# NikNazarov/TorchPIV

Hardware: AMD Instinct MI355X
Metric: image-pairs/sec at 4 MP, wind=64 ov=32 2-pass CWS; % HBM roofline (higher is better)
Workload: dtype u32 exact sums + f64 / f32

## Files before the change

torchpiv_amd/csrc/xcorr_tile.hpp:

```cpp
#pragma once
#include <hip/hip_runtime.h>
#include <stdint.h>

#include "fft_inreg.hpp"
#include "piv_kernels.h"

namespace tpiv {

template <int WS, bool PLANAR_ = false>
struct TileGeo {
    static constexpr int WPW = 64 / WS;
    static constexpr int TS = WS > 32 ? 32 : WS;
    static constexpr int PITCH = TS + 1;
    static constexpr int NT = 64 / TS;
    static constexpr int TILE = TS * PITCH;
    static constexpr bool PLANAR = PLANAR_;
    static constexpr int HROWS = WS / 2 + 1;
    static constexpr int HTILE = HROWS * PITCH;
    static constexpr int LDS_FLOATS = NT * TILE * (PLANAR ? 1 : 2);
    static constexpr int MAP_PITCH = WS + 1;
    static constexpr int NDW = WS / 4;
};

template <int CTRL>
// ... 709 lines not shown
                if (ci < CG::T) {
                    pa[j * CG::PITCH4 + part] = make_uint4(raw.ca[k][0], raw.ca[k][1], raw.ca[k][2], raw.ca[k][3]);
                    pb[j * CG::PITCH4 + part] = make_uint4(raw.cb[k][0], raw.cb[k][1], raw.cb[k][2], raw.cb[k][3]);
                }
            }
            wave_sync();
            const int rlo = -8, rhi = p.H + 7;
            const float gy0f = (float)g.y0;
            const int base_a = clamp_i(f2i_sat_t(floorf(gy0f - vy)), rlo, rhi);
            const int base_b = clamp_i(f2i_sat_t(floorf(gy0f + vy)), rlo, rhi);
            const uint4* s0 = pa + (clamp_i(c.dya, rlo, rhi) - base_a) * CG::PITCH4;
            const uint4* s1 = pa + (clamp_i(c.uya, rlo, rhi) - base_a) * CG::PITCH4;
            const uint4* s2 = pb + (clamp_i(c.dyb, rlo, rhi) - base_b) * CG::PITCH4;
            const uint4* s3 = pb + (clamp_i(c.uyb, rlo, rhi) - base_b) * CG::PITCH4;
            auto fetch = [&](const uint4* src, uint32_t (&d)[NB]) TPIV_LAMBDA_INLINE {
#pragma unroll
                for (int q = 0; q < NB / 4; ++q) {
                    const uint4 t = src[q];
                    d[4 * q] = t.x, d[4 * q + 1] = t.y, d[4 * q + 2] = t.z, d[4 * q + 3] = t.w;
                }
                static_assert(CG::RPG * 4 >= NB, "patch rows hold the whole 16-byte unit of the last dword");
                d[NB - 1] = read_unit_x(src + NB / 4);
            };
            if (raw.fix) {
                constexpr int LAST = CG::LOADED / 4 - 1;
                auto fix_lds = [&](const uint4* src, int cls) TPIV_LAMBDA_INLINE {
                    if (cls != 0) {
                        const uint32_t* sw = reinterpret_cast<const uint32_t*>(src);
                        const uint32_t px = (cls == 1 ? (sw[0] & 0xffu) : (sw[LAST] >> 24)) * 0x01010101u;
                        uint4* dst = const_cast<uint4*>(src);
#pragma unroll
                        for (int q = 0; q < CG::RPG; ++q) dst[q] = make_uint4(px, px, px, px);
                    }
                };
                fix_lds(s0, raw.cls & 3);
                fix_lds(s1, (raw.cls >> 2) & 3);
                fix_lds(s2, (raw.cls >> 4) & 3);
                fix_lds(s3, (raw.cls >> 6) & 3);
                wave_sync();
            }
            constexpr bool LAZY = FAST && WS == 64;
            if constexpr (LAZY) {
                lz0 = s0, lz1 = s1, lz2 = s2, lz3 = s3;
            } else {
                fetch(s0, ra0);
                fetch(s1, ra1);
                fetch(s2, rb0);
                fetch(s3, rb1);
            }
            float4* wbuf = reinterpret_cast<float4*>(lds + CG::FLOATS) + (lane / WS) * (WS + 1);
            {
                const float gxf = gx0f + (float)r;
                const float nxa = gxf - vx, nxb = gxf + vx;
                const float uxa_f = ceilf(nxa), dxa_f = floorf(nxa);
                const float uxb_f = ceilf(nxb), dxb_f = floorf(nxb);
                wave_sync();
                wbuf[r] = make_float4(uxa_f - nxa, nxa - dxa_f, uxb_f - nxb, nxb - dxb_f);
                wave_sync();
            }
            if constexpr (FAST) {
                constexpr bool LAZY = WS == 64;
                auto pull = [&](auto qc) TPIV_LAMBDA_INLINE {
                    constexpr int q = decltype(qc)::value;
                    auto one = [&](const uint4* src, uint32_t (&d)[NB]) TPIV_LAMBDA_INLINE {
                        if constexpr (4 * q + 3 < NB) {
                            const uint4 t = src[q];
                            d[4 * q] = t.x, d[4 * q + 1] = t.y, d[4 * q + 2] = t.z, d[4 * q + 3] = t.w;
                        } else {
                            d[NB - 1] = read_unit_x(src + NB / 4);
                        }
                    };
                    one(lz0, ra0), one(lz1, ra1), one(lz2, rb0), one(lz3, rb1);
                };
                if constexpr (LAZY) {
                    pull(std::integral_constant<int, 0>{});
                    pull(std::integral_constant<int, 1>{});
                }
                auto row_lerp = [&](auto kc, const uint32_t (&r0_)[NB], const uint32_t (&r1_)[NB], float wu_, float wd_) TPIV_LAMBDA_INLINE {
                    constexpr int k = decltype(kc)::value;
                    return fmaf(byte_f<k, NB>(r1_), wd_, byte_f<k, NB>(r0_) * wu_);
                };
                float va = row_lerp(std::integral_constant<int, 0>{}, ra0, ra1, c.wya_up, c.wya_dn);
                float vb = row_lerp(std::integral_constant<int, 0>{}, rb0, rb1, c.wyb_up, c.wyb_dn);
                static_for<0, WS>([&](auto kc) TPIV_LAMBDA_INLINE {
                    constexpr int k = decltype(kc)::value;
                    if constexpr (k % 8 == 0 && k > 0) __builtin_amdgcn_sched_barrier(0);
                    if constexpr (LAZY && k % 16 == 0 && k > 0) pull(std::integral_constant<int, k / 16 + 1>{});
                    const float4 wx = wbuf[k];
                    const float na = row_lerp(std::integral_constant<int, k + 1>{}, ra0, ra1, c.wya_up, c.wya_dn);
                    const float nb = row_lerp(std::integral_constant<int, k + 1>{}, rb0, rb1, c.wyb_up, c.wyb_dn);
#ifdef TPIV_MUTANT_LERP
                    x[k].x = fmaf(na, wx.y * 1.001f, va * wx.x);
#else
                    x[k].x = fmaf(na, wx.y, va * wx.x);
#endif
                    x[k].y = fmaf(nb, wx.w, vb * wx.z);
                    va = na;
                    vb = nb;
                });
            } else {
            unsigned dmask_a = c.ydeg_a ? ~0u : 0u, dmask_b = c.ydeg_b ? ~0u : 0u;
            asm volatile("" : "+v"(dmask_a), "+v"(dmask_b));
            static_for<0, WS>([&](auto kc) TPIV_LAMBDA_INLINE {
                constexpr int k = decltype(kc)::value;
                if constexpr (k % 8 == 0 && k > 0) __builtin_amdgcn_sched_barrier(0);
                const float4 wx = wbuf[k];
                x[k].x = bilerp_ref_m(byte_f<k, NB>(ra0), byte_f<k + 1, NB>(ra0), byte_f<k, NB>(ra1),
                                      byte_f<k + 1, NB>(ra1), wx.x, wx.y, c.wya_up, c.wya_dn, dmask_a);
                x[k].y = bilerp_ref_m(byte_f<k, NB>(rb0), byte_f<k + 1, NB>(rb0), byte_f<k, NB>(rb1),
                                      byte_f<k + 1, NB>(rb1), wx.z, wx.w, c.wyb_up, c.wyb_dn, dmask_b);
            });
            }
            wave_sync();
        } else {
            wave_sync();
            static_for<0, RBH>([&](auto hc) TPIV_LAMBDA_INLINE {
            constexpr int k0 = decltype(hc)::value * RBL;
#pragma unroll UNR_CWS
            for (int k = 0; k < RBL; ++k) {
                const float nxa = (gx0f + (float)(k0 + k)) - vx;
                const float uxa_f = ceilf(nxa), dxa_f = floorf(nxa);
                const int uxa = f2i_sat_t(uxa_f), dxa = f2i_sat_t(dxa_f);
                rowbuf[k] = bilerp_ref(fetch_clamped_t(fa, (long long)c.dya * p.W + dxa, HW),
                                       fetch_clamped_t(fa, (long long)c.dya * p.W + uxa, HW),
                                       fetch_clamped_t(fa, (long long)c.uya * p.W + dxa, HW),
                                       fetch_clamped_t(fa, (long long)c.uya * p.W + uxa, HW), uxa_f - nxa,
                                       nxa - dxa_f, c.wya_up, c.wya_dn, c.ydeg_a || (uxa == dxa));
            }
#pragma unroll
            for (int k = 0; k < RBL; ++k) x[k0 + k].x = rowbuf[k];
#pragma unroll UNR_CWS
            for (int k = 0; k < RBL; ++k) {
                const float nxb = (gx0f + (float)(k0 + k)) + vx;
                const float uxb_f = ceilf(nxb), dxb_f = floorf(nxb);
                const int uxb = f2i_sat_t(uxb_f), dxb = f2i_sat_t(dxb_f);
                rowbuf[k] = bilerp_ref(fetch_clamped_t(fb, (long long)c.dyb * p.W + dxb, HW),
                                       fetch_clamped_t(fb, (long long)c.dyb * p.W + uxb, HW),
                                       fetch_clamped_t(fb, (long long)c.uyb * p.W + dxb, HW),
                                       fetch_clamped_t(fb, (long long)c.uyb * p.W + uxb, HW), uxb_f - nxb,
                                       nxb - dxb_f, c.wyb_up, c.wyb_dn, c.ydeg_b || (uxb == dxb));
            }
#pragma unroll
            for (int k = 0; k < RBL; ++k) x[k0 + k].y = rowbuf[k];
            });
            wave_sync();
        }
        sa = 0.f;
        sb = 0.f;
        if constexpr (!FAST) {
#pragma unroll
            for (int k = 0; k < WS; ++k) {
                sa += x[k].x;
                sb += x[k].y;
            }
        }
    }
}

template <int WS>
__device__ __forceinline__ unsigned long long exclusion_row_mask(int m, int ys, int wv) {
    static_assert(WS <= 64, "one 64-bit mask per row");
    const int my_ = m / WS, mx_ = m % WS, KD = WS * WS;
    const int dj = ys - my_;
    unsigned long long ex = 0ull;
    auto span = [&](int lo_, int hi_) TPIV_LAMBDA_INLINE {
        lo_ = lo_ < 0 ? 0 : lo_;
        hi_ = hi_ > WS - 1 ? WS - 1 : hi_;
        if (lo_ > hi_) return 0ull;
        const unsigned long long ones = (hi_ - lo_ + 1) >= 64 ? ~0ull : ((1ull << (hi_ - lo_ + 1)) - 1ull);
        return ones << lo_;
    };
    if (dj >= -wv && dj <= wv) ex |= span(mx_ - wv, mx_ + wv);
    if (dj + 1 >= -wv && dj + 1 <= wv) ex |= span(mx_ - wv + WS, mx_ + wv + WS);
    if (dj - 1 >= -wv && dj - 1 <= wv) ex |= span(mx_ - wv - WS, mx_ + wv - WS);
    if (ys == 0 && (m - wv - wv * WS) <= 0) ex |= 1ull;
    if (ys == WS - 1 && (m + wv + wv * WS) >= KD - 1) ex |= 1ull << (WS - 1);
    return ex;
}

__device__ __forceinline__ float max3_skip_nan(float a, float b, float c) {
    float o;
    asm("v_max3_f32 %0, %1, %2, %3" : "=v"(o) : "v"(a), "v"(b), "v"(c));
    return o;
}
__device__ __forceinline__ float max_skip_nan(float a, float b) {
    float o;
    asm("v_max_f32 %0, %1, %2" : "=v"(o) : "v"(a), "v"(b));
    return o;
}

template <int WS, bool PLANAR, bool SCALED = false>
__device__ __forceinline__ void peak_analysis(const PassParams& p, const float (&row)[WS], float* tile, int w, int r,
                                              bool active, bool dead, size_t fidx, float scale = 1.0f) {
    using G = TileGeo<WS, PLANAR>;
    constexpr bool SMALLMAP = G::WPW * WS * G::MAP_PITCH > G::LDS_FLOATS;
    static_assert(G::WPW * 3 * G::MAP_PITCH <= G::LDS_FLOATS, "map rows must fit the tile LDS");
    float* my_map = tile + w * ((SMALLMAP ? 3 : WS) * G::MAP_PITCH);
    const int ys = (r + WS / 2) % WS;
    float cmin = 3.4e38f, rraw = -3.4e38f;
#pragma unroll
    for (int k = 0; k < WS; ++k) {
        cmin = fminf(cmin, row[k]);
        rraw = fmaxf(rraw, row[k]);
    }
    cmin = grp_min<WS>(cmin);
    const float ncs = -(cmin * scale);
    auto shifted = [&](float c_) TPIV_LAMBDA_INLINE {
        if constexpr (SCALED) return __fadd_rn(fmaf(c_, scale, ncs), 1e-7f);
        else return __fadd_rn(__fsub_rn(c_, cmin), 1e-7f);
    };
    if constexpr (!SMALLMAP) {
        static_for<0, WS>([&](auto kc) TPIV_LAMBDA_INLINE {
            constexpr int xsft = decltype(kc)::value;
            my_map[ys * G::MAP_PITCH + xsft] = row[(xsft + WS / 2) % WS];
        });
    }
    const float rmax = shifted(rraw);
    const float gmax = grp_reduce<WS>(rmax, [](float a, float b) TPIV_LAMBDA_INLINE { return fmaxf(a, b); });
    auto imin = [](int a, int b) TPIV_LAMBDA_INLINE { return a < b ? a : b; };
    const int ywin = grp_reduce<WS>(rmax == gmax ? ys : WS - 1, imin);
    const int row0 = SMALLMAP ? ywin - 1 : 0;
    if constexpr (SMALLMAP) {
        wave_sync();
        const int slot = ys - row0;
        if (slot >= 0 && slot <= 2) {
            static_for<0, WS>([&](auto kc) TPIV_LAMBDA_INLINE {
                constexpr int xsft = decltype(kc)::value;
                my_map[slot * G::MAP_PITCH + xsft] = row[(xsft + WS / 2) % WS];
            });
        }
    }
    wave_sync();

    if (p.dbg_corr != nullptr && active) {
        int yy = ys;
        asm volatile("" : "+v"(yy));
        float* d = p.dbg_corr + fidx * WS * WS + yy * WS;
        static_for<0, WS>([&](auto kc) TPIV_LAMBDA_INLINE {
            constexpr int xsft = decltype(kc)::value;
            d[xsft] = shifted(row[(xsft + WS / 2) % WS]);
        });
    }
    const int xwin = grp_reduce<WS>(shifted(my_map[(ywin - row0) * G::MAP_PITCH + r]) == gmax ? r : WS - 1, imin);

    const int m = ywin * WS + xwin;
    const int KD = WS * WS;
    const int wv = p.val_win;
    float sraw;
    {
        const unsigned long long ex = exclusion_row_mask<WS>(m, ys, wv);
        const int exl = (int)(unsigned)ex, exh = (int)(unsigned)(ex >> 32);
        float acc = __int_as_float(-1);
        static_for<0, WS / 2>([&](auto kc) TPIV_LAMBDA_INLINE {
            constexpr int x0 = 2 * decltype(kc)::value, x1 = x0 + 1;
            const int k0 = __builtin_amdgcn_sbfe(x0 < 32 ? exl : exh, x0 & 31, 1);
            const int k1 = __builtin_amdgcn_sbfe(x1 < 32 ? exl : exh, x1 & 31, 1);
            const float v0 = __int_as_float(__float_as_int(row[(x0 + WS / 2) % WS]) | k0);
            const float v1 = __int_as_float(__float_as_int(row[(x1 + WS / 2) % WS]) | k1);
            acc = max3_skip_nan(acc, v0, v1);
        });
        sraw = acc;
    }
    sraw = grp_reduce<WS>(sraw, [](float a, float b) TPIV_LAMBDA_INLINE { return max_skip_nan(a, b); });
    const float second_v = sraw != sraw ? gmax : shifted(sraw);

    {
        int left = m + 1, right = m - 1, top = m + WS, bot = m - WS;
        if (left >= KD - 1) left = m;
        if (right <= 0) right = m;
        if (top >= KD - 1) top = m;
        if (bot <= 0) bot = m;
        int q = m;
        q = (r == 1) ? left : q;
        q = (r == 2) ? right : q;
        q = (r == 3) ? top : q;
        q = (r == 4) ? bot : q;
        float outv = shifted(my_map[(q / WS - row0) * G::MAP_PITCH + (q % WS)]);
        outv = (r == 5) ? second_v : outv;
        outv = (r == 6) ? __int_as_float(m) : outv;
        outv = (r == 7) ? __int_as_float(dead ? 1 : 0) : outv;
        if (r < 8 && active) p.peak_raw[fidx * 8 + r] = outv;
    }
}



template <int WS>
__device__ __forceinline__ void peak_candidates(const PassParams& p, const float (&row)[WS], float* tile, int w, int r,
                                                bool active, bool dead, size_t fidx, float band_abs) {
    static_assert(WS == 8 || WS == 16 || WS == 32 || WS == 64, "64 / WS windows per wavefront");
    auto wballot = [&](bool pred) TPIV_LAMBDA_INLINE {
        const unsigned long long b_ = __ballot(pred);
        if constexpr (WS == 64) return b_;
        else return (b_ >> (w * WS)) & ((1ull << WS) - 1ull);
    };
    auto any_left = [](unsigned long long mk) TPIV_LAMBDA_INLINE {
        if constexpr (WS == 64) return mk != 0ull;
        else return __ballot(mk != 0ull) != 0ull;
    };
    auto mine_left = [](unsigned long long mk) TPIV_LAMBDA_INLINE {
        if constexpr (WS == 64) return true;
        else return mk != 0ull;
    };
    float* const my_row = tile + w * WS;
    const int ys = (r + WS / 2) % WS;
    if (p.dbg_corr != nullptr && active) {
        int yy = ys;
        asm volatile("" : "+v"(yy));
        float* d = p.dbg_corr + fidx * WS * WS + yy * WS;
        static_for<0, WS>([&](auto kc) TPIV_LAMBDA_INLINE {
            constexpr int xsft = decltype(kc)::value;
            d[xsft] = row[(xsft + WS / 2) % WS];
        });
    }
    float rmin = 3.4e38f, rmax = -3.4e38f;
#pragma unroll
    for (int k = 0; k < WS; ++k) {
        rmin = fminf(rmin, row[k]);
        rmax = fmaxf(rmax, row[k]);
    }
    const float cmin = grp_min<WS>(rmin);
    const float gmax = grp_reduce<WS>(rmax, [](float a, float b) TPIV_LAMBDA_INLINE { return fmaxf(a, b); });
    const float band = fmaxf(p.exact_band_range * (gmax - cmin), band_abs);
    bool open = !(band > 0.0f) || !(gmax > cmin);
    auto park = [&](int rl) TPIV_LAMBDA_INLINE {
        wave_sync();
        if (r == rl) {
#pragma unroll
            for (int k = 0; k < WS; ++k) my_row[(k + WS / 2) % WS] = row[k];
        }
        wave_sync();
        return my_row[r];
    };
    auto row_of_lane = [](int rl) TPIV_LAMBDA_INLINE { return (rl + WS / 2) % WS; };
    int m = 0;
    {
        const unsigned long long rows = wballot(rmax >= gmax - band);
        open = open || __popcll(rows) != 1;
        const int rl = rows ? (int)__builtin_ctzll(rows) : 0;
        const unsigned long long cols = wballot(park(rl) >= gmax - band);
        open = open || __popcll(cols) != 1;
        m = row_of_lane(rl) * WS + (cols ? (int)__builtin_ctzll(cols) : 0);
    }
    const int wv = p.val_win;
    int s[EXACT_MAX_SECOND] = {-1, -1, -1};
    {
        const unsigned long long ex = exclusion_row_mask<WS>(m, ys, wv);
        const int exl = (int)(unsigned)ex, exh = (int)(unsigned)(ex >> 32);
        int smax = -1;
        static_for<0, WS>([&](auto kc) TPIV_LAMBDA_INLINE {
            constexpr int xsft = decltype(kc)::value;
            constexpr int xo = (xsft + WS / 2) % WS;
            const int kill = __builtin_amdgcn_sbfe(xsft < 32 ? exl : exh, xsft & 31, 1);
            const int cnd = __float_as_int(__fsub_rn(row[xo], cmin)) | kill;
            smax = cnd > smax ? cnd : smax;
        });
        const int sall = grp_reduce<WS>(smax, [](int a, int b) TPIV_LAMBDA_INLINE { return a > b ? a : b; });
        const float thr = __int_as_float(sall) - band;
        unsigned long long rows = sall >= 0 ? wballot(smax >= 0 && __int_as_float(smax) >= thr) : 0ull;
        open = open || __popcll(rows) > EXACT_MAX_SECOND;
        int ns = 0;
        for (int it = 0; it < EXACT_MAX_SECOND; ++it) {
            if (!any_left(rows)) break;
            const bool on = mine_left(rows);
            const int rl = on ? (int)__builtin_ctzll(rows) : 0;
            rows &= rows - 1;
            const int yr = row_of_lane(rl);
            const unsigned long long exr = exclusion_row_mask<WS>(m, yr, wv);
            unsigned long long cols = wballot(__fsub_rn(park(rl), cmin) >= thr) & ~exr;
            cols = on ? cols : 0ull;
            for (int k = 0; k < WS; ++k) {
                if (!any_left(cols)) break;
                const bool has = mine_left(cols);
                const int q = yr * WS + (has ? (int)__builtin_ctzll(cols) : 0);
                cols &= cols - 1;
                s[0] = (has && ns == 0) ? q : s[0];
                s[1] = (has && ns == 1) ? q : s[1];
                s[2] = (has && ns == 2) ? q : s[2];
                ns += has ? 1 : 0;
            }
        }
        open = open || ns > EXACT_MAX_SECOND;
    }
    int n[EXACT_MAX_MIN] = {-1, -1, -1, -1};
    {
        const float thr = cmin + band;
        unsigned long long rows = wballot(rmin <= thr);
        bool over = __popcll(rows) > EXACT_MAX_MIN;
        int nn = 0;
        for (int it = 0; it < EXACT_MAX_MIN; ++it) {
            if (!any_left(rows)) break;
            const bool on = mine_left(rows);
            const int rl = on ? (int)__builtin_ctzll(rows) : 0;
            rows &= rows - 1;
            const int yr = row_of_lane(rl);
            unsigned long long cols = wballot(park(rl) <= thr);
            cols = on ? cols : 0ull;
            over = over || nn + __popcll(cols) > EXACT_MAX_MIN;
            for (int k = 0; k < EXACT_MAX_MIN; ++k) {
                if (!any_left(cols)) break;
                const bool has = mine_left(cols) && cols != 0ull && nn < EXACT_MAX_MIN;
                const int q = yr * WS + (cols ? (int)__builtin_ctzll(cols) : 0);
                cols &= cols - 1;
                n[0] = (has && nn == 0) ? q : n[0];
                n[1] = (has && nn == 1) ? q : n[1];
                n[2] = (has && nn == 2) ? q : n[2];
                n[3] = (has && nn == 3) ? q : n[3];
                nn += has ? 1 : 0;
            }
        }
        n[3] = over ? -2 : n[3];
    }
    if (r == 0 && active) {
        const int m_out = dead ? -2 : (open ? -1 : m);
        auto pack = [](int lo_, int hi_) TPIV_LAMBDA_INLINE { return ((unsigned)lo_ & 0xffffu) | ((unsigned)hi_ << 16); };
        uint4 rec;
        rec.x = pack(m_out, s[0]);
        rec.y = pack(s[1], s[2]);
        rec.z = pack(n[0], n[1]);
        rec.w = pack(n[2], n[3]);
        p.cand[fidx] = rec;
    }
}

template <int WS, int MODE, int OCC, bool FAST, bool CAND, int ROLE = 0>
__device__ __forceinline__ void xcorr_tile_body(const PassParams& p) {
    constexpr bool PLANAR = OCC > 2;
    using G = TileGeo<WS, PLANAR>;
    static_assert(WS == 8 || WS == 16 || WS == 32 || WS == 64, "tile sizes of this kernel");
    constexpr int RBH = 64 * (WS + 1) <= G::LDS_FLOATS ? 1 : 2;
    static_assert(MODE == MODE_PASS1 || 64 * (WS / RBH + 1) <= G::LDS_FLOATS,
                  "slow-path row buffer (shifted passes) must fit the tile LDS");
    constexpr int LDSF = (MODE == MODE_CWS && CoopGeo<WS>::LDS_FLOATS > G::LDS_FLOATS)
                             ? CoopGeo<WS>::LDS_FLOATS : G::LDS_FLOATS;
    __shared__ __attribute__((aligned(16))) float tile[LDSF];

    using TW = std::conditional_t<WS == 16, TwRegs<WS>, TwLiteral>;
    TW tw;
    if constexpr (!std::is_same<TW, TwLiteral>::value) tw.init();

    const int N = p.n_rows * p.n_cols;
    const int groups = (N + G::WPW - 1) / G::WPW;
    const bool listed = ROLE == 0 && MODE != MODE_PASS1 && p.list_mode != 0;
    const int items = listed ? __builtin_amdgcn_readfirstlane((int)*p.slow_count) : p.batch * groups;
    const int st = p.ws - p.ov;
    auto real_item = [&](int pos) TPIV_LAMBDA_INLINE { return listed ? __builtin_amdgcn_readfirstlane(p.slow_list[pos]) : pos; };

    constexpr int QCH = WS <= 16 ? 4 : 1;
    const int xcd = blockIdx.x & 7;
    const int chunk = (int)(((long long)items + 7) / 8);
    const int lo = __builtin_amdgcn_readfirstlane(xcd * chunk < items ? xcd * chunk : items);
    const int hi = __builtin_amdgcn_readfirstlane(items - lo > chunk ? lo + chunk : items);
    unsigned* const ctr = p.work_ctr + xcd * 16;
    int q_base = 0;
    int q_left = 0;
    auto q_issue = [&]() TPIV_LAMBDA_INLINE -> unsigned {
        unsigned v = 0;
        if (QCH == 1 || q_left == 0) {
            if (fresh_lane() == 0) v = atomicAdd(ctr, (unsigned)QCH);
        }
        return v;
    };
    auto q_take = [&](unsigned q_raw) TPIV_LAMBDA_INLINE -> int {
        if (QCH == 1 || q_left == 0) {
            const unsigned v = (unsigned)__builtin_amdgcn_readfirstlane((int)q_raw);
            q_base = v < (unsigned)(hi - lo) ? lo + (int)v : hi;
            q_left = QCH;
        }
        const int it = q_base + (QCH - q_left);
        --q_left;
        return it;
    };

    auto geom_of = [&](int pos, int w) TPIV_LAMBDA_INLINE {
        ItemGeom g;
        const int item = real_item(pos);
        g.pair = fast_div(item, p.groups_magic, p.groups_shift);
        const int gi = item - g.pair * groups;
        const int win_raw = gi * G::WPW + w;
        g.active = win_raw < N ? 1 : 0;
        g.win = g.active ? win_raw : N - 1;
        const int wrow = fast_div(g.win, p.ncols_magic, p.ncols_shift);
        g.y0 = wrow * st;
        g.x0 = (g.win - wrow * p.n_cols) * st;
        g.fidx = (size_t)g.pair * N + g.win;
        return g;
    };
    auto shift_of = [&](const ItemGeom& g, float& vx, float& vy) TPIV_LAMBDA_INLINE {
        if constexpr (MODE == MODE_PASS1) {
            vx = 0.f;
            vy = 0.f;
        } else {
            if constexpr (MODE == MODE_CWS) {
                pred_half_shift_cws_f32(p, g.fidx, vx, vy);
            } else {
                double sx, sy;
                pred_half_shift<MODE>(p, g.fidx, sx, sy);
                vx = (float)sx;
                vy = (float)sy;
            }
        }
    };

    int item = q_take(q_issue());
    if (item >= hi) return;
    int nitem = q_take(q_issue());
    constexpr bool RECOMPUTE = WS >= 32;
    float vx, vy;
    RawRows<WS, MODE> raw;
    ItemGeom gcur;
    CoopOff<WS> coff;
    if constexpr (MODE == MODE_CWS) coff.init(fresh_lane() % WS, p.W);
    {
        const int l0 = fresh_lane();
        gcur = geom_of(item, l0 / WS);
        shift_of(gcur, vx, vy);
        issue_rows<WS, MODE, FAST>(p, gcur, l0 % WS, vx, vy, raw, coff);
    }

    TPIV_STAMP_DECL
    TPIV_STAMP_START;
    for (int nnitem; item < hi; item = nitem, nitem = nnitem) {
        const unsigned q_raw = q_issue();
#ifdef TPIV_STAMPS
        ++st_iter;
#endif
        const int lane = fresh_lane();
        const int w = lane / WS;
        const int r = lane % WS;
        const ItemGeom g = RECOMPUTE ? geom_of(item, w) : gcur;
        const bool active = g.active != 0;
        const size_t fidx = g.fidx;
        const int nit = nitem < hi ? nitem : item;
        const ItemGeom gnext = geom_of(nit, w);
        float nvx, nvy;
        shift_of(gnext, nvx, nvy);

        if constexpr (ROLE == 1) {
            if (!raw.reg) {
                if (lane == 0) p.slow_list[atomicAdd(p.slow_count, 1u)] = item;
                nnitem = q_take(q_raw);
                issue_rows<WS, MODE, FAST>(p, gnext, r, nvx, nvy, raw, coff);
                vx = nvx;
                vy = nvy;
                if constexpr (!RECOMPUTE) gcur = gnext;
                continue;
            }
        }
        cf x[WS];
        float sa, sb;
        constexpr int NBS = WS >= 32 ? G::WPW : 1;
        int band_s[NBS];
        TPIV_STAMP(0);
        RowSquares sq;
        convert_rows<WS, MODE, RBH, FAST, CAND, ROLE == 1 ? 1 : 0>(p, g, r, lane, vx, vy, raw, x, sa, sb, tile, &sq);
        TPIV_STAMP(1);
        if constexpr (WS >= 64) nnitem = q_take(q_raw);
        if constexpr (WS <= 32) issue_rows<WS, MODE, FAST>(p, gnext, r, nvx, nvy, raw, coff);

        if (p.dbg_win != nullptr && active) {
            int rr = r;
            asm volatile("" : "+v"(rr));
            float* d = p.dbg_win + fidx * 2 * WS * WS + rr * WS;
#pragma unroll
            for (int k = 0; k < WS; ++k) {
                d[k] = x[k].x;
                d[WS * WS + k] = x[k].y;
            }
        }

        bool dead = false;
        float end_scale = 1.0f;
        constexpr bool FASTN = FAST && MODE != MODE_PASS1;
        constexpr bool NOSWAP = WS == 64 && !(MODE == MODE_DWS && FAST);
        auto up_sign = []() TPIV_LAMBDA_INLINE { return fresh_lane() >= 32 ? 0x80000000u : 0u; };
        auto sflip = [](float v, unsigned sg) TPIV_LAMBDA_INLINE { return __uint_as_float(__float_as_uint(v) ^ sg); };
        if constexpr (!FASTN) {
            sa = grp_sum<WS>(sa);
            sb = grp_sum<WS>(sb);
            const float ma = sa * (1.0f / (WS * WS)), mb = sb * (1.0f / (WS * WS));
            float ka = 1.f, kb = 1.f;
            if constexpr (MODE == MODE_PASS1) {
                dead = (sa == 0.f) || (sb == 0.f);
                ka = dead ? 0.f : 1.0f / ma;
                kb = dead ? 0.f : 1.0f / mb;
            }
            if constexpr (CAND) {
                auto uadd = [](unsigned a_, unsigned b_) TPIV_LAMBDA_INLINE { return a_ + b_; };
                const unsigned saa = grp_reduce<WS>(sq.aa, uadd), sbb = grp_reduce<WS>(sq.bb, uadd);
                constexpr double NN = (double)(WS * WS);
                const double da = (double)sa, db = (double)sb;
                const float ea = (float)__fma_rn(-da, da, NN * (double)saa), eb = (float)__fma_rn(-db, db, NN * (double)sbb);
                const float e_plus = (0.5f / (float)(WS * WS)) * (ea * (ka * ka) + eb * (kb * kb));
                const float bnd = dead ? 0.f : p.exact_band * e_plus;
                if constexpr (WS >= 32) {
                    static_for<0, G::WPW>([&](auto wc) TPIV_LAMBDA_INLINE {
                        band_s[decltype(wc)::value] = __builtin_amdgcn_readlane(__float_as_int(bnd), decltype(wc)::value * WS);
                    });
                } else {
                    band_s[0] = __float_as_int(bnd);
                }
            }
            constexpr float PRE = 0.5f / (float)WS;
            const float oa = -ma * ka, ob = -mb * kb;
            const float kas = ka * PRE, kbs = kb * PRE, oas = oa * PRE, obs = ob * PRE;
            const unsigned sg = NOSWAP ? up_sign() : 0u;
            const float kao = sflip(kas, sg), kbo = sflip(kbs, sg), oao = sflip(oas, sg), obo = sflip(obs, sg);
#pragma unroll
            for (int k = 0; k < WS; ++k) {
                x[k].x = (k & 1) ? fmaf(x[k].x, kao, oao) : fmaf(x[k].x, kas, oas);
                x[k].y = (k & 1) ? fmaf(x[k].y, kbo, obo) : fmaf(x[k].y, kbs, obs);
            }
        } else if constexpr (NOSWAP) {
            const unsigned sg = up_sign();
#pragma unroll
            for (int k = 1; k < WS; k += 2) {
                x[k].x = sflip(x[k].x, sg);
                x[k].y = sflip(x[k].y, sg);
            }
        }

        TPIV_STAMP(2);
        fft_inreg<WS, 1>(x, tw);
        if constexpr (FASTN) {
            constexpr int P0 = FFT_POS<0, WS>;
            if constexpr (NOSWAP) {
                constexpr int PH = FFT_POS<WS / 2, WS>;
                const bool up = up_sign() != 0u;
                const float ta = grp_sum<WS>(up ? x[PH].x : x[P0].x);
                const float tb = grp_sum<WS>(up ? x[PH].y : x[P0].y);
                x[P0].x -= up ? 0.0f : ta * (1.0f / WS);
                x[P0].y -= up ? 0.0f : tb * (1.0f / WS);
                x[PH].x -= up ? ta * (1.0f / WS) : 0.0f;
                x[PH].y -= up ? tb * (1.0f / WS) : 0.0f;
            } else {
                const float ta = grp_sum<WS>(x[P0].x);
                const float tb = grp_sum<WS>(x[P0].y);
                x[P0].x -= ta * (1.0f / WS);
                x[P0].y -= tb * (1.0f / WS);
            }
            end_scale = 0.25f / (float)(WS * WS);
        }
        TPIV_STAMP(3);
        transpose_tile<WS, PLANAR, NOSWAP>(x, tile, fresh_lane());
        TPIV_STAMP(4);
        fft_inreg<WS, 1>(x, tw);
        TPIV_STAMP(5);

        constexpr bool HALF_INV = PLANAR && (WS == 32 || WS == 64);
        float crow[WS];
        if constexpr (HALF_INV) {
            constexpr int M = WS / 2;
            cf h[M];
            {
                const int lane_c = fresh_lane();
                const int r_c = lane_c % WS;
                const int partner = (lane_c - r_c) + ((WS - r_c) % WS);
                auto cross = [&](cf zk, cf zm, float two) TPIV_LAMBDA_INLINE {
                    const float a_ = zk.x, b_ = zk.y, c_ = zm.x, d_ = zm.y;
                    cf pr;
                    pr.x = (a_ * d_ + b_ * c_) * two;
                    pr.y = (c_ * c_ - a_ * a_) + (d_ * d_ - b_ * b_);
                    return pr;
                };
                const float two_odd = (NOSWAP && (lane_c & 31) != 0) ? -2.0f : 2.0f;
                cf pc[M + 1];
                static_for<0, M + 1>([&](auto kc) TPIV_LAMBDA_INLINE {
                    constexpr int ky = decltype(kc)::value;
                    constexpr int nky = (WS - ky) % WS;
                    const cf z2 = x[FFT_POS<nky, WS>];
                    cf m1;
                    m1.x = __shfl(z2.x, partner, 64);
                    m1.y = __shfl(z2.y, partner, 64);
                    pc[ky] = cross(x[FFT_POS<ky, WS>], m1, (ky & 1) ? two_odd : 2.0f);
                });
                TPIV_STAMP(6);
                const bool odd = r_c > M;
                const float fs = (r_c == 0 || r_c == M) ? 1.0f : 0.0f;
                static_for<0, M>([&](auto kc) TPIV_LAMBDA_INLINE {
                    constexpr int k = decltype(kc)::value;
                    cf pr;
                    pr.x = __shfl(pc[M - k].x, partner, 64);
                    pr.y = __shfl(pc[M - k].y, partner, 64);
                    const cf s{pc[k].x + pr.x, pc[k].y - pr.y};
                    const cf tt = twmul<k, WS, -1>(cf{pc[k].x - pr.x, pc[k].y + pr.y});
                    h[k].x = odd ? tt.x : __builtin_fmaf(-fs, tt.y, s.x);
                    h[k].y = odd ? tt.y : __builtin_fmaf(fs, tt.x, s.y);
                });
            }
            fft_inreg<M, -1>(h, tw);
            TPIV_STAMP(7);
            cf hs[M + 1], z[M];
            transpose_half_pairs<WS, PLANAR>(h, hs, tile, fresh_lane());
            TPIV_STAMP(8);
            c2r_inreg<WS>(hs, z);
            static_for<0, WS>([&](auto xc) TPIV_LAMBDA_INLINE {
                constexpr int x_ = decltype(xc)::value;
                crow[x_] = (x_ & 1) ? z[FFT_POS<x_ / 2, M>].y : z[FFT_POS<x_ / 2, M>].x;
            });
        } else {
            {
                const int lane_c = fresh_lane();
                const int r_c = lane_c % WS;
                const int partner = (lane_c - r_c) + ((WS - r_c) % WS);
                auto cross = [&](cf zk, cf zm, float two) TPIV_LAMBDA_INLINE {
                    const float a_ = zk.x, b_ = zk.y, c_ = zm.x, d_ = zm.y;
                    cf pr;
                    pr.x = (a_ * d_ + b_ * c_) * two;
                    pr.y = (c_ * c_ - a_ * a_) + (d_ * d_ - b_ * b_);
                    return pr;
                };
                const float two_odd = (NOSWAP && (lane_c & 31) != 0) ? -2.0f : 2.0f;
                static_for<0, WS / 2 + 1>([&](auto kc) TPIV_LAMBDA_INLINE {
// ... 186 lines not shown
```

Baseline: 18750.

## Batch candidate-row parking into LDS slots to cut per-row wave syncs

Peak-candidate search previously parked one correlation row at a time into LDS, with two wave syncs per probed row across the max, second-peak and minimum searches. Now all minimum-candidate rows plus the max row are written at once into per-window slots with float4 stores, and all column ballots are taken after a single sync pair. Second-peak rows are handled the same way in a second batch. The loops are unrolled with static_for. This cuts sync and LDS round trips in exchange for more LDS slot space and more registers for the precomputed column masks.

Result: no change. 18770, median of 5 (+0.1%).

```diff
diff --git a/torchpiv_amd/csrc/xcorr_tile.hpp b/torchpiv_amd/csrc/xcorr_tile.hpp
--- a/torchpiv_amd/csrc/xcorr_tile.hpp
+++ b/torchpiv_amd/csrc/xcorr_tile.hpp
@@ -1035,7 +1035,6 @@
         if constexpr (WS == 64) return true;
         else return mk != 0ull;
     };
-    float* const my_row = tile + w * WS;
     const int ys = (r + WS / 2) % WS;
     if (p.dbg_corr != nullptr && active) {
         int yy = ys;
@@ -1056,22 +1055,40 @@
     const float gmax = grp_reduce<WS>(rmax, [](float a, float b) TPIV_LAMBDA_INLINE { return fmaxf(a, b); });
     const float band = fmaxf(p.exact_band_range * (gmax - cmin), band_abs);
     bool open = !(band > 0.0f) || !(gmax > cmin);
-    auto park = [&](int rl) TPIV_LAMBDA_INLINE {
-        wave_sync();
-        if (r == rl) {
-#pragma unroll
-            for (int k = 0; k < WS; ++k) my_row[(k + WS / 2) % WS] = row[k];
-        }
-        wave_sync();
-        return my_row[r];
+    constexpr int SLOT = WS + 4, NSLOT = 1 + EXACT_MAX_MIN;
+    static_assert(EXACT_MAX_SECOND <= NSLOT, "trip B reuses the slots of trip A");
+    static_assert((64 / WS) * NSLOT * SLOT <= TileGeo<WS, true>::LDS_FLOATS, "slot areas must fit the (planar) tile LDS");
+    float* const my_slots = tile + w * (NSLOT * SLOT);
+    auto below = [](unsigned long long mk, int l) TPIV_LAMBDA_INLINE { return (int)__popcll(mk & ((1ull << l) - 1ull)); };
+    auto bit = [](unsigned long long mk, int l) TPIV_LAMBDA_INLINE { return ((mk >> l) & 1ull) != 0ull; };
+    auto park_rows = [&](int slot) TPIV_LAMBDA_INLINE {
+        wave_sync();
+        if (slot >= 0) {
+            float* const d = my_slots + slot * SLOT;
+            static_for<0, WS / 4>([&](auto jc) TPIV_LAMBDA_INLINE {
+                constexpr int k = 4 * decltype(jc)::value;
+                *reinterpret_cast<float4*>(d + (k + WS / 2) % WS) = make_float4(row[k], row[k + 1], row[k + 2], row[k + 3]);
+            });
+        }
+        wave_sync();
     };
     auto row_of_lane = [](int rl) TPIV_LAMBDA_INLINE { return (rl + WS / 2) % WS; };
+    const float hi = gmax - band, thr_n = cmin + band;
+    const unsigned long long rows_n = wballot(rmin <= thr_n);
     int m = 0;
+    unsigned long long cols_n[EXACT_MAX_MIN];
     {
-        const unsigned long long rows = wballot(rmax >= gmax - band);
+        const unsigned long long rows = wballot(rmax >= hi);
         open = open || __popcll(rows) != 1;
         const int rl = rows ? (int)__builtin_ctzll(rows) : 0;
-        const unsigned long long cols = wballot(park(rl) >= gmax - band);
+        const int slot_m = (bit(rows_n, rl) && below(rows_n, rl) < EXACT_MAX_MIN) ? 1 + below(rows_n, rl) : 0;
+        const int rk = below(rows_n, r);
+        park_rows((bit(rows_n, r) && rk < EXACT_MAX_MIN) ? 1 + rk : (r == rl ? 0 : -1));
+        const unsigned long long cols = wballot(my_slots[slot_m * SLOT + r] >= hi);
+        static_for<0, EXACT_MAX_MIN>([&](auto ic) TPIV_LAMBDA_INLINE {
+            constexpr int it = decltype(ic)::value;
+            cols_n[it] = wballot(my_slots[(1 + it) * SLOT + r] <= thr_n);
+        });
         open = open || __popcll(cols) != 1;
         m = row_of_lane(rl) * WS + (cols ? (int)__builtin_ctzll(cols) : 0);
     }
@@ -1092,56 +1109,66 @@
         const float thr = __int_as_float(sall) - band;
         unsigned long long rows = sall >= 0 ? wballot(smax >= 0 && __int_as_float(smax) >= thr) : 0ull;
         open = open || __popcll(rows) > EXACT_MAX_SECOND;
+        unsigned long long cols_s[EXACT_MAX_SECOND] = {0ull, 0ull, 0ull};
+        if (any_left(rows)) {
+            const int rk = below(rows, r);
+            park_rows((bit(rows, r) && rk < EXACT_MAX_SECOND) ? rk : -1);
+            static_for<0, EXACT_MAX_SECOND>([&](auto ic) TPIV_LAMBDA_INLINE {
+                constexpr int it = decltype(ic)::value;
+                cols_s[it] = wballot(__fsub_rn(my_slots[it * SLOT + r], cmin) >= thr);
+            });
+        }
         int ns = 0;
-        for (int it = 0; it < EXACT_MAX_SECOND; ++it) {
-            if (!any_left(rows)) break;
-            const bool on = mine_left(rows);
-            const int rl = on ? (int)__builtin_ctzll(rows) : 0;
-            rows &= rows - 1;
-            const int yr = row_of_lane(rl);
-            const unsigned long long exr = exclusion_row_mask<WS>(m, yr, wv);
-            unsigned long long cols = wballot(__fsub_rn(park(rl), cmin) >= thr) & ~exr;
-            cols = on ? cols : 0ull;
-            for (int k = 0; k < WS; ++k) {
-                if (!any_left(cols)) break;
-                const bool has = mine_left(cols);
-                const int q = yr * WS + (has ? (int)__builtin_ctzll(cols) : 0);
-                cols &= cols - 1;
-                s[0] = (has && ns == 0) ? q : s[0];
-                s[1] = (has && ns == 1) ? q : s[1];
-                s[2] = (has && ns == 2) ? q : s[2];
-                ns += has ? 1 : 0;
-            }
-        }
+        static_for<0, EXACT_MAX_SECOND>([&](auto ic) TPIV_LAMBDA_INLINE {
+            constexpr int it = decltype(ic)::value;
+            if (any_left(rows)) {
+                const bool on = mine_left(rows);
+                const int rl = on ? (int)__builtin_ctzll(rows) : 0;
+                rows &= rows - 1;
+                const int yr = row_of_lane(rl);
+                const unsigned long long exr = exclusion_row_mask<WS>(m, yr, wv);
+                unsigned long long cols = on ? (cols_s[it] & ~exr) : 0ull;
+                for (int k = 0; k < WS; ++k) {
+                    if (!any_left(cols)) break;
+                    const bool has = mine_left(cols);
+                    const int q = yr * WS + (has ? (int)__builtin_ctzll(cols) : 0);
+                    cols &= cols - 1;
+                    s[0] = (has && ns == 0) ? q : s[0];
+                    s[1] = (has && ns == 1) ? q : s[1];
+                    s[2] = (has && ns == 2) ? q : s[2];
+                    ns += has ? 1 : 0;
+                }
+            }
+        });
         open = open || ns > EXACT_MAX_SECOND;
     }
     int n[EXACT_MAX_MIN] = {-1, -1, -1, -1};
     {
-        const float thr = cmin + band;
-        unsigned long long rows = wballot(rmin <= thr);
+        unsigned long long rows = rows_n;
         bool over = __popcll(rows) > EXACT_MAX_MIN;
         int nn = 0;
-        for (int it = 0; it < EXACT_MAX_MIN; ++it) {
-            if (!any_left(rows)) break;
-            const bool on = mine_left(rows);
-            const int rl = on ? (int)__builtin_ctzll(rows) : 0;
-            rows &= rows - 1;
-            const int yr = row_of_lane(rl);
-            unsigned long long cols = wballot(park(rl) <= thr);
-            cols = on ? cols : 0ull;
-            over = over || nn + __popcll(cols) > EXACT_MAX_MIN;
-            for (int k = 0; k < EXACT_MAX_MIN; ++k) {
-                if (!any_left(cols)) break;
-                const bool has = mine_left(cols) && cols != 0ull && nn < EXACT_MAX_MIN;
-                const int q = yr * WS + (cols ? (int)__builtin_ctzll(cols) : 0);
-                cols &= cols - 1;
-                n[0] = (has && nn == 0) ? q : n[0];
-                n[1] = (has && nn == 1) ? q : n[1];
-                n[2] = (has && nn == 2) ? q : n[2];
-                n[3] = (has && nn == 3) ? q : n[3];
-                nn += has ? 1 : 0;
-            }
-        }
+        static_for<0, EXACT_MAX_MIN>([&](auto ic) TPIV_LAMBDA_INLINE {
+            constexpr int it = decltype(ic)::value;
+            if (any_left(rows)) {
+                const bool on = mine_left(rows);
+                const int rl = on ? (int)__builtin_ctzll(rows) : 0;
+                rows &= rows - 1;
+                const int yr = row_of_lane(rl);
+                unsigned long long cols = on ? cols_n[it] : 0ull;
+                over = over || nn + __popcll(cols) > EXACT_MAX_MIN;
+                for (int k = 0; k < EXACT_MAX_MIN; ++k) {
+                    if (!any_left(cols)) break;
+                    const bool has = mine_left(cols) && cols != 0ull && nn < EXACT_MAX_MIN;
+                    const int q = yr * WS + (cols ? (int)__builtin_ctzll(cols) : 0);
+                    cols &= cols - 1;
+                    n[0] = (has && nn == 0) ? q : n[0];
+                    n[1] = (has && nn == 1) ? q : n[1];
+                    n[2] = (has && nn == 2) ? q : n[2];
+                    n[3] = (has && nn == 3) ? q : n[3];
+                    nn += has ? 1 : 0;
+                }
+            }
+        });
         n[3] = over ? -2 : n[3];
     }
     if (r == 0 && active) {
```
